# algbio/GraphChainer

Measured on AMD Instinct MI355X. Metric: reads_per_sec, higher is better.
Workload: dtype u64

## Files before the change

### graphchainer_amd/csrc/hip/gc_device.hpp

```cpp
#pragma once
#include <hip/hip_runtime.h>
#include <stdint.h>

#ifndef GC_LOOP_TICK
#define GC_LOOP_TICK(i) ((void)0)
#endif

namespace gcdev {

struct NodeRec {
	uint32_t comp;
	uint32_t outOff;
	uint32_t inOff;
	uint32_t meta;
	uint64_t w0, w1;
};
enum : uint32_t { NODEREC_SLOW = 128u };

struct DGraph {
	uint32_t nNodes;
	uint32_t firstAmbiguous;
	const uint8_t*  nodeLength;
	const uint32_t* nodeOffset;
	const int32_t*  nodeIDs;
	const uint64_t* nodeSeq;
	const uint64_t* ambSeq;
	const uint32_t* inOff;  const uint32_t* inAdj;
	const uint32_t* outOff; const uint32_t* outAdj;
	const uint32_t* componentNumber;
	const uint32_t* origSize;
	const uint32_t* lookupOff;
	const uint32_t* lookup;
	const uint32_t* componentMap;
	const uint32_t* topoId;
	const uint32_t* pathsOff; const uint32_t* paths; const uint32_t* pathsPos;
	const uint32_t* backOff;  const uint32_t* backNode; const uint32_t* backPath; const uint32_t* backPos;
	const uint32_t* mpcWidth;
	const uint32_t* chainNumber;
	const uint64_t* chainApproxPos;
	const NodeRec* nodeRec;
};

struct WS {
	uint64_t VP, VN;
	int32_t score;
};

__device__ __forceinline__ int popc64(uint64_t x) { return __popcll(x); }
__device__ __forceinline__ int32_t wsBefore(const WS& w) { return w.score - popc64(w.VP) + popc64(w.VN); }
__device__ __forceinline__ int32_t wsValue(const WS& w, int row)
{
	uint64_t above = row < 63 ? (~0ull << (row + 1)) : 0ull;
	return w.score + popc64(w.VN & above) - popc64(w.VP & above);
}

__device__ inline WS wsMerge(const WS& a, const WS& b)
{
	int32_t d = wsBefore(a) - wsBefore(b);
	uint64_t takeB = 0, fixP = 0, fixN = 0, fixMask = 0;
	uint64_t diff = (a.VP ^ b.VP) | (a.VN ^ b.VN);
	int pos = 0;
	while (diff) {
		GC_LOOP_TICK(0);
		int r = __ffsll((long long)diff) - 1;
		diff &= diff - 1;
		uint64_t bit = 1ull << r;
		if (d > 0 && r > pos) takeB |= (bit - 1) & ~((1ull << pos) - 1);
		int da = (int)((a.VP >> r) & 1) - (int)((a.VN >> r) & 1);
		int db = (int)((b.VP >> r) & 1) - (int)((b.VN >> r) & 1);
		int nd = d + da - db;
		bool before = d > 0, after = nd > 0;
		if (before != after) {
			int delta = after ? (db - d) : (da + d);
			fixMask |= bit;
			if (delta > 0) fixP |= bit;
// ... 175 lines not shown
	uint32_t startBit;
	__device__ __forceinline__ void rows(int len, int j, Eq4& eq) const;
};
__device__ inline void eqVectorBits(const EqSource& src, int len, int j, Eq4& eq)
{
	int n = len - j;
	if (n > 64) n = 64;
	uint32_t bit = src.startBit + (uint32_t)j;
	uint32_t w = bit >> 6, sh = bit & 63;
	uint64_t keep = n >= 64 ? ~0ull : ((1ull << n) - 1);
	uint64_t out[4];
	for (int b = 0; b < 4; b++) {
		const uint64_t* v = src.masks + (size_t)b * src.words;
		uint64_t lo = v[w] >> sh;
		uint64_t hi = (sh != 0 && w + 1 < src.words) ? (v[w + 1] << (64 - sh)) : 0ull;
		out[b] = (lo | hi) & keep;
	}
	eq.a = out[0]; eq.c = out[1]; eq.g = out[2]; eq.t = out[3];
}
__device__ __forceinline__ void EqSource::rows(int len, int j, Eq4& eq) const { eqVectorBits(*this, len, j, eq); }

struct NodeSeq { uint64_t w0, w1, w2, w3; bool ambiguous; };
__device__ __forceinline__ NodeSeq loadNodeSeq(const DGraph& g, uint32_t node)
{
	NodeSeq s;
	if (node < g.firstAmbiguous) {
		s.w0 = g.nodeSeq[2 * (size_t)node];
		s.w1 = g.nodeSeq[2 * (size_t)node + 1];
		s.w2 = s.w3 = 0;
		s.ambiguous = false;
	} else {
		const uint64_t* p = g.ambSeq + 4 * (size_t)(node - g.firstAmbiguous);
		s.w0 = p[0]; s.w1 = p[1]; s.w2 = p[2]; s.w3 = p[3];
		s.ambiguous = true;
	}
	return s;
}
__device__ __forceinline__ uint64_t eqOfColumn(const Eq4& eq, const NodeSeq& s, int pos)
{
	if (!s.ambiguous) {
		uint64_t w = pos < 32 ? s.w0 : s.w1;
		uint32_t code = (uint32_t)(w >> ((pos & 31) * 2));
		uint64_t lo = (code & 1) ? eq.c : eq.a;
		uint64_t hi = (code & 1) ? eq.t : eq.g;
		return (code & 2) ? hi : lo;
	}
	uint64_t r = 0;
	r |= ((s.w0 >> pos) & 1) ? eq.a : 0ull;
	r |= ((s.w1 >> pos) & 1) ? eq.c : 0ull;
	r |= ((s.w2 >> pos) & 1) ? eq.g : 0ull;
	r |= ((s.w3 >> pos) & 1) ? eq.t : 0ull;
	return r;
}

__device__ inline int findItem(const uint32_t* itemNodes, const SliceInfo& sl, uint32_t node)
{
	for (uint32_t i = 0; i < sl.count; i++)
		if (itemNodes[sl.first + i] == node) return (int)(sl.first + i);
	return -1;
}

__device__ __forceinline__ int32_t clipXScore(int32_t cells, int32_t scoreHere, double errorCost)
{
#pragma clang fp contract(off)
	const double product = (double)scoreHere * errorCost;
	const double difference = (double)cells - product;
// ... 586 lines not shown
```

### graphchainer_amd/csrc/hip/gc_device_wave.hpp

```cpp
#pragma once
#include "gc_device.hpp"
#include "gc_column_asm.hpp"
#include <type_traits>

namespace gcdev {


#ifndef WAVE_CAP
#define WAVE_CAP 28
#endif

#define WAVE_ENTRY_WORDS 7
#define WAVE_WORDS (3 * WAVE_CAP * WAVE_ENTRY_WORDS)
template <int LANES> struct WaveLdsT { uint32_t w[WAVE_WORDS][LANES]; };
typedef WaveLdsT<64> WaveLds;
static_assert(sizeof(WaveLds) <= 160 * 1024, "WaveLds must fit the CU's LDS");
static_assert(64 * 5 <= WAVE_WORDS, "the 64 backtrace columns (5 words each) alias the lane's table words");

#define WAVE_SPILL 228
#define WAVE_MAX_ENTRIES (WAVE_CAP + WAVE_SPILL)
#define WAVE_SPILL_WORDS (3 * WAVE_SPILL * 4)

typedef __attribute__((address_space(3))) uint32_t lds_u32;

// ... 268 lines not shown
	const int32_t beforeMin = beforeA < beforeB ? beforeA : beforeB;
	int32_t above = __builtin_amdgcn_update_dpp(0, m, 0x138, 0xf, 0xf, false);
	if (threadIdx.x == 0) above = beforeMin;
	WS res;
	res.VP = __ballot(m == above + 1);
	res.VN = __ballot(m == above - 1);
	res.score = a.score < b.score ? a.score : b.score;
	return res;
}
#endif

struct TilePreamble { uint64_t prevHP, prevHN, forceEq; int forceUntil; };
template <bool ROWS_IN_LANES>
__device__ __forceinline__ int32_t clipMaxXScoreWave(const WS& w, double errorCost)
{
#if defined(__HIP_DEVICE_COMPILE__)
	if (ROWS_IN_LANES) {
		const uint64_t upTo = ~(~1ull << threadIdx.x);
		const int32_t value = wsBefore(w) + popc64(w.VP & upTo) - popc64(w.VN & upTo);
		int32_t x = clipXScore((int32_t)threadIdx.x + 1, value, errorCost);
		auto higher = [](int32_t a, int32_t b) { return a > b ? a : b; };
		x = higher(x, __builtin_amdgcn_update_dpp(INT32_MIN, x, 0x111, 0xf, 0xf, false));
		x = higher(x, __builtin_amdgcn_update_dpp(INT32_MIN, x, 0x112, 0xf, 0xf, false));
		x = higher(x, __builtin_amdgcn_update_dpp(INT32_MIN, x, 0x114, 0xf, 0xf, false));
		x = higher(x, __builtin_amdgcn_update_dpp(INT32_MIN, x, 0x118, 0xf, 0xf, false));
		x = higher(x, __builtin_amdgcn_update_dpp(INT32_MIN, x, 0x142, 0xa, 0xf, false));
		x = higher(x, __builtin_amdgcn_update_dpp(INT32_MIN, x, 0x143, 0xc, 0xf, false));
		return (int32_t)GC_READLANE(x, 63);
	}
#endif
	return clipMaxXScore(w, errorCost, 64);
}
template <int MODE, bool CLIP = false, typename LANE_TABLES>
__device__ __forceinline__ TileResult computeTileW(const DGraph& g, uint32_t node, WS ws, bool prevExists, int32_t prevStartScore, uint64_t prevHP, uint64_t prevHN,
	const Eq4& eq, NodeItem& out, const LANE_TABLES& tables, int flatRows, uint32_t& status, TilePreamble* preambleOnly = nullptr, double errorCost = 0, int32_t* maxX = nullptr)
{
	constexpr bool COLUMNS = MODE == 1;
	int nodeLength = g.nodeLength[node];
	NodeSeq seq = loadNodeSeq(g, node);
	TileResult r;
	r.minScore = ws.score;
	r.minOffset = 0;
	if (CLIP && maxX) *maxX = clipMaxXScoreWave<LANE_TABLES::eqInLanes>(ws, errorCost);
#if defined(__HIP_DEVICE_COMPILE__)
	if (prevExists && wsBefore(ws) > prevStartScore) ws = LANE_TABLES::eqInLanes ? wsMergeWave(ws, wsSource(prevStartScore)) : wsMerge(ws, wsSource(prevStartScore));
#else
	if (prevExists && wsBefore(ws) > prevStartScore) ws = wsMerge(ws, wsSource(prevStartScore));
#endif
	int forceUntil = 0;
	if (prevExists) {
		int32_t scoreBefore = wsBefore(ws);
		int32_t scoreComparison = prevStartScore;
		if (scoreBefore > scoreComparison) status = EXT_ASSERT;
		if (scoreBefore < scoreComparison) {
			for (int fix = 1; fix < 64; fix++) {
				int32_t next = scoreComparison + (int32_t)((prevHP >> fix) & 1) - (int32_t)((prevHN >> fix) & 1);
				uint64_t mask = 1ull << fix;
				if (scoreBefore > next) status = EXT_ASSERT;
				if (scoreBefore < next) { prevHP |= mask; prevHN &= ~mask; forceUntil = fix; }
				if (scoreBefore == next) { prevHP &= ~mask; prevHN &= ~mask; }
				scoreBefore++;
				scoreComparison = next;
				if (scoreBefore >= scoreComparison) break;
			}
		}
	} else {
		forceUntil = nodeLength;
	}
	out.node = node;
	out.sVP = ws.VP; out.sVN = ws.VN; out.sScore = ws.score;
	uint64_t flatMask = flatRows > 0 ? ~(~0ull << flatRows) : 0;
	r.flatMin = INT32_MAX;
// ... 59 lines not shown
		if (ws.score < r.minScore) { r.minScore = ws.score; r.minOffset = (uint32_t)pos; }
		if (flatRows > 0) {
			int32_t f = ws.score - popc64(ws.VP & ~flatMask) + popc64(ws.VN & ~flatMask);
			if (f < r.flatMin) { r.flatMin = f; r.flatOffset = (uint32_t)pos; }
		}
		if (MODE != 0) tables.colSet((uint32_t)pos, ws);
		if (CLIP && maxX) { const int32_t x = clipMaxXScoreWave<LANE_TABLES::eqInLanes>(ws, errorCost); *maxX = x > *maxX ? x : *maxX; }
		HP |= hp << pos;
		HN |= hn << pos;
	}
	out.HP = HP; out.HN = HN;
	out.eVP = ws.VP; out.eVN = ws.VN; out.eScore = ws.score;
	return r;
}


template <bool REGCOLS, bool BAND = false, bool CLIP = false>
__device__ __forceinline__ uint32_t extendSeedWave(const DGraph& g, const CorrectnessTables& ct, const EqSource& eqSrc, int bandwidthCfg, lds_u32* lds, const WaveScratch& wsx,
	int len, uint32_t startNode, uint32_t startOffset, uint32_t which, uint32_t& nTrace, int32_t& score, ExtCounters& cnt, int rampBandwidth = 0, uint32_t maxCells = ~0u, bool forceGlobal = false,
	double errorCost = 0, int32_t xDrop = 0)
{
	static_assert(BAND || !CLIP, "CLIP is instantiated with BAND");
	const LaneLdsT<REGCOLS> L { lds, wsx.lane, wsx.lanes, wsx.spillBase(), {}, wsx.regCap < 64 ? wsx.regCap : 64u, { 0, 0, 0, 0, 0 }, 0, 0 };
	uint32_t status = EXT_OK;
	nTrace = 0;
	score = 0;
	cnt.extensions++;
	cnt.flattenTie = 0;
	int numSlices = (len + 63) / 64;
	if ((uint32_t)numSlices + 1 > wsx.maxSlices) return EXT_OVERFLOW;
	int buf = 0;
	uint32_t nPrev = 1;
	{
		int nl = g.nodeLength[startNode];
		NodeItem it;
		it.node = startNode;
		it.sVP = it.sVN = it.eVP = it.eVN = 0;
		it.sScore = (int32_t)startOffset;
		it.eScore = nl - 1 - (int32_t)startOffset;
		it.minScore = 0;
		uint64_t upToOffset = startOffset >= 63 ? ~0ull : ((1ull << (startOffset + 1)) - 1);
		uint64_t nodeMask = nl >= 64 ? ~0ull : ((1ull << nl) - 1);
		it.HN = upToOffset & ~1ull;
		it.HP = nodeMask & ~upToOffset;
		storeItem(wsx, 0, it);
		L.pSet(0, 0, startNode, it.sScore, 0, it.HP, it.HN);
		WSlice s0;
		s0.minScore = 0; s0.minNode = startNode; s0.minOffset = startOffset; s0.first = 0; s0.count = 1; s0.bandwidth = 1; s0.j = -64; s0.flags = 1;
		if (CLIP) setClipScore(s0, startNode, 0);
		storeSlice(wsx, 0, s0);
	}
	uint32_t nItems = 1, nSlices = 1;
	const bool storeCols = REGCOLS && wsx.maxCols > 0;
	uint32_t nCols = 0;
	GC_MARK_START();
	int32_t prevMinScore = 0, prevBandwidth = 1, prevJ = -64;
	double prevCorrect = ct.initCorrect, prevFalse = ct.initFalse;
	int rampUntil = 0, rampRedoIndex = -1;
	const bool rampOn = BAND && rampBandwidth > bandwidthCfg;
	const bool keepAll = BAND && forceGlobal;
	double snapCorrect = 0, snapFalse = 0;
	uint32_t snapCols = 0;
	const bool xDropOn = CLIP && xDrop > 0;
	int32_t bestXScore = 0;
	Eq4 eq;
	for (int slice = 0; slice < numSlices; slice++) {
		int j = prevJ + 64;
		eqVectorBits(eqSrc, len, j, eq);
		int32_t previousQuitScore = prevMinScore + prevBandwidth;
		int bandwidth = bandwidthCfg;
		if (BAND && rampOn && rampUntil >= slice && !xDropOn) bandwidth = rampBandwidth;
		const uint32_t sliceCols = nCols;
		uint32_t cells = 0;
		int flatRows = (!CLIP && j + 64 > len) ? (len - j) : 0;
		int32_t sliceMaxX = INT32_MIN; uint32_t sliceMaxXNode = 0xffffffffu;
		const int cb = REGCOLS ? 1 : (buf ^ 1);
		auto prevFind = [&](uint32_t node) __attribute__((always_inline)) -> int { return L.find((uint32_t)(REGCOLS ? 0 : buf), nPrev, node); };
		uint32_t nPending = 0;
		auto pushEdge = [&](uint32_t target, WS incoming, bool skipFirst) __attribute__((always_inline)) {
			int found = L.find(2u, nPending, target);
			uint32_t slot = found >= 0 ? (uint32_t)found : nPending;
			WS add = incoming;
			if (!skipFirst) {
				int pi = prevFind(target);
				bool prevExists = pi >= 0;
				int32_t prevStart = prevExists ? L.pStart(buf, (uint32_t)pi) : 0;
				uint64_t hinP, hinN;
				if (prevExists) {
					int32_t before = wsBefore(incoming);
					if (prevStart < before) { hinP = 0; hinN = 1; }
					else if (prevStart > before) { hinP = 1; hinN = 0; }
					else { hinP = 0; hinN = 0; }
				} else { hinP = 1; hinN = 0; }
				NodeSeq nseq = loadNodeSeq(g, target);
				uint64_t hp, hn;
#if defined(__HIP_DEVICE_COMPILE__)
				uint64_t eqFirst;
				if (REGCOLS && !nseq.ambiguous) {
					uint64_t lo, hi;
					const uint32_t code = (uint32_t)__builtin_amdgcn_readfirstlane((int)(uint32_t)nseq.w0);
					const uint64_t mA = gcUniform64(eq.a), mC = gcUniform64(eq.c), mG = gcUniform64(eq.g), mT = gcUniform64(eq.t);
					asm("s_bitcmp1_b32 %3, 0\n\ts_cselect_b64 %0, %5, %4\n\ts_cselect_b64 %1, %7, %6\n\ts_bitcmp1_b32 %3, 1\n\ts_cselect_b64 %2, %1, %0"
						: "=&s"(lo), "=&s"(hi), "=&s"(eqFirst) : "s"(code), "s"(mA), "s"(mC), "s"(mG), "s"(mT) : "scc");
				} else eqFirst = eqOfColumn(eq, nseq, 0);
				add = myersStep(eqFirst, incoming, hinP, hinN, hp, hn);
#else
				add = myersStep(eqOfColumn(eq, nseq, 0), incoming, hinP, hinN, hp, hn);
#endif
				if (!prevExists || wsBefore(add) < prevStart) { add.VP &= ~1ull; add.VN |= 1ull; }
			}
			if (slot == nPending) {
				if (nPending >= L.maxEntries()) { status = EXT_LDS_CAP; return; }
				L.qSet(slot, target, g.componentNumber[target], add);
				nPending++;
			} else {
#if defined(__HIP_DEVICE_COMPILE__)
				L.qSetWs(slot, REGCOLS ? wsMergeWave(L.qWs(slot), add) : wsMerge(L.qWs(slot), add));
#else
				L.qSetWs(slot, wsMerge(L.qWs(slot), add));
#endif
			}
		};
		for (uint32_t i = 0; i < nPrev; i++) {
			if (j != 0 && L.pMin(buf, i) > previousQuitScore) continue;
			pushEdge(L.pNode(buf, i), wsSource(L.pStart(buf, i)), true);
		}
		if (status != EXT_OK) return status;
		GC_MARK(0);
		WSlice cur;
		cur.first = nItems; cur.count = 0; cur.bandwidth = bandwidth; cur.j = j;
		cur.minScore = INT32_MAX - bandwidth - 1; cur.minNode = 0xffffffffu; cur.minOffset = 0xffffffffu;
		int32_t flatMin = INT32_MAX; uint32_t flatNode = 0xffffffffu, flatOffset = 0xffffffffu;
		int32_t currentMin = cur.minScore;
		while (nPending > 0) {
			const uint32_t best = L.qArgMin(nPending);
			uint32_t pnode = L.qNode(best);
			WS pws = L.qWs(best);
			if (best != nPending - 1) L.qMove(best, nPending - 1);
			nPending--;
			if (nItems >= wsx.maxItems) return EXT_OVERFLOW;
			if (cur.count >= L.maxEntries()) return EXT_LDS_CAP;
			int pi = prevFind(pnode);
			bool prevExists = pi >= 0;
			NodeItem out;
			typename LaneLdsT<REGCOLS>::Entry pe { 0, 0, 0, ~0ull, 0ull };
			if (prevExists) pe = L.get((uint32_t)buf, (uint32_t)pi);
			GC_MARK(1);
			const uint32_t tileLength = g.nodeLength[pnode];
			if (storeCols && nCols + tileLength - 1 > wsx.maxCols) return EXT_OVERFLOW;
			int32_t tileMaxX = INT32_MIN;
			TileResult tr = storeCols ? computeTileW<2, CLIP>(g, pnode, pws, prevExists, (int32_t)pe.w1, pe.a, pe.b, eq, out, L, flatRows, status, nullptr, errorCost, CLIP ? &tileMaxX : nullptr)
				: computeTileW<0, CLIP>(g, pnode, pws, prevExists, (int32_t)pe.w1, pe.a, pe.b, eq, out, L, flatRows, status, nullptr, errorCost, CLIP ? &tileMaxX : nullptr);
			GC_MARK(2);
			if (status != EXT_OK) return status;
			if (CLIP && tileMaxX > sliceMaxX) { sliceMaxX = tileMaxX; sliceMaxXNode = pnode; }
			out.minScore = tr.minScore;
			if (storeCols) {
				if (threadIdx.x >= 1 && threadIdx.x < tileLength) {
					ulonglong2 v;
					v.x = (unsigned long long)L.cr[0] | ((unsigned long long)L.cr[1] << 32);
					v.y = (unsigned long long)L.cr[2] | ((unsigned long long)L.cr[3] << 32);
					*(ulonglong2*)(wsx.base + wsx.colBase() + 2ull * (nCols + threadIdx.x - 1)) = v;
				}
				NodeItem stored = out;
				stored.minScore = (int32_t)nCols;
				storeItem(wsx, nItems, stored);
				nCols += tileLength - 1;
			} else storeItem(wsx, nItems, out);
			L.pSet(cb, cur.count, pnode, out.sScore, out.minScore, out.HP, out.HN);
			nItems++;
			cur.count++;
			cnt.dpTiles++;
			cnt.columnSteps += g.nodeLength[pnode];
			if (flatRows > 0) { cnt.recomputeTiles++; cnt.columnSteps += g.nodeLength[pnode]; }
			if (tr.minScore > previousQuitScore + bandwidth + 128) return EXT_ASSERT;
			currentMin = tr.minScore < currentMin ? tr.minScore : currentMin;
			if (tr.minScore < cur.minScore) { cur.minScore = tr.minScore; cur.minNode = pnode; cur.minOffset = tr.minOffset; }
			if (flatRows > 0) {
				if (tr.flatMin < flatMin) { flatMin = tr.flatMin; flatNode = pnode; flatOffset = tr.flatOffset; }
				else if (tr.flatMin == flatMin) flatOffset |= 0x80000000u;
			}
			WS newEnd = itemEnd(out);
#if defined(__HIP_DEVICE_COMPILE__)
			int32_t newEndMin;
			if (REGCOLS) {
				const uint64_t upTo = ~(~1ull << threadIdx.x);
				const int32_t before = wsBefore(newEnd);
				uint32_t v = (uint32_t)(before + popc64(newEnd.VP & upTo) - popc64(newEnd.VN & upTo));
				auto lower = [](uint32_t a, uint32_t b) { return (int32_t)a < (int32_t)b ? a : b; };
				v = lower(v, (uint32_t)__builtin_amdgcn_update_dpp(0x7fffffff, (int)v, 0x111, 0xf, 0xf, false));
				v = lower(v, (uint32_t)__builtin_amdgcn_update_dpp(0x7fffffff, (int)v, 0x112, 0xf, 0xf, false));
				v = lower(v, (uint32_t)__builtin_amdgcn_update_dpp(0x7fffffff, (int)v, 0x114, 0xf, 0xf, false));
				v = lower(v, (uint32_t)__builtin_amdgcn_update_dpp(0x7fffffff, (int)v, 0x118, 0xf, 0xf, false));
				v = lower(v, (uint32_t)__builtin_amdgcn_update_dpp(0x7fffffff, (int)v, 0x142, 0xa, 0xf, false));
				v = lower(v, (uint32_t)__builtin_amdgcn_update_dpp(0x7fffffff, (int)v, 0x143, 0xc, 0xf, false));
				const int32_t rowsMin = (int32_t)GC_READLANE(v, 63);
				newEndMin = rowsMin < before ? rowsMin : before;
			} else newEndMin = wsColumnMin(newEnd);
#else
			int32_t newEndMin = wsColumnMin(newEnd);
#endif
			if (newEndMin < prevMinScore) return EXT_ASSERT;
			if (newEndMin <= currentMin + bandwidth) {
				GC_MARK(3);
				for (uint32_t e = g.outOff[pnode]; e < g.outOff[pnode + 1]; e++) {
					pushEdge(g.outAdj[e], newEnd, false);
					if (status != EXT_OK) return status;
				}
				GC_MARK(4);
			} else GC_MARK(3);
			if (BAND) {
				cells += tileLength;
				if (cells > maxCells) break;
			}
		}
		GC_MARK(1);
		if (cur.count == 0) return EXT_ASSERT;
		const uint32_t flatTie = flatRows > 0 ? (flatOffset >> 31) << 3 : 0u;
		if (flatRows > 0) { cur.minScore = flatMin; cur.minNode = flatNode; cur.minOffset = flatOffset & 0x7fffffffu; }
		if (cur.minScore < prevMinScore) return EXT_ASSERT;
		if (CLIP) setClipScore(cur, sliceMaxXNode, sliceMaxX + j);
		double curCorrect, curFalse;
		{
			int mm = cur.minScore - prevMinScore;
			int idx = mm < 64 ? mm : 63;
			bool cfc = prevCorrect + ct.c2c >= prevFalse + ct.f2c;
			bool ffc = prevCorrect + ct.c2f >= prevFalse + ct.f2f;
			double a = prevCorrect + ct.c2c, b = prevFalse + ct.f2c;
			double c = prevCorrect + ct.c2f, d = prevFalse + ct.f2f;
			curCorrect = (a > b ? a : b) + ct.correctOdds[idx];
			curFalse = (c > d ? c : d) + ct.wrongOdds[idx];
			cur.flags = (curCorrect > curFalse ? 1u : 0u) | (cfc ? 2u : 0u) | (ffc ? 4u : 0u) | flatTie;
		}
		if (BAND) {
			if (!keepAll && !xDropOn && (rampUntil == slice - 1 || (rampUntil < slice && (cur.flags & 1u) && (cur.flags & 4u)))) {
				if (nPrev > wsx.maxTrace) return EXT_OVERFLOW;
				rampRedoIndex = slice - 1;
				snapCorrect = prevCorrect; snapFalse = prevFalse; snapCols = sliceCols;
				for (uint32_t i = 0; i < nPrev; i++) { const int32_t mn = L.pMin(buf, i); if (wsx.storer()) wsx.word(wsx.traceBase(i, which)) = (unsigned long long)(uint32_t)mn; }
// ... 70 lines not shown
		if (REGCOLS) {
			const bool mine = threadIdx.x == (nTrace & 63u);
			tbLo = mine ? (uint32_t)cell : tbLo;
			tbHi = mine ? (uint32_t)(cell >> 32) : tbHi;
			nTrace++;
			if ((nTrace & 63u) == 0) flushTrace(64);
		} else {
			wsx.word(wsx.traceBase(nTrace, which)) = cell;
			nTrace++;
		}
		return true;
	};
	Cell here { last.minNode, last.minOffset, (last.j + 63 < len - 1) ? last.j + 63 : len - 1 };
	if (CLIP) {
		uint32_t bestIndex = 1;
		WSlice bs = loadSlice(wsx, 1);
		for (uint32_t k = 2; k < nSlices; k++) { const WSlice t = loadSlice(wsx, k); if (clipScore(t) > clipScore(bs)) { bs = t; bestIndex = k; } }
		const uint32_t bestNode = clipNode(bs);
		const int bestItem = findItemW(wsx, bs, bestNode);
		if (bestItem < 0) return EXT_ASSERT;
		const NodeItem it = loadItem(wsx, (uint32_t)bestItem);
		const int prevIdx = findItemW(wsx, loadSlice(wsx, bestIndex - 1), bestNode);
		const bool prevExists = prevIdx >= 0;
		NodeItem pit {};
		if (prevExists) pit = loadItem(wsx, (uint32_t)prevIdx);
		eqVectorBits(eqSrc, len, bs.j, eq);
		ClipFind find { clipScore(bs) - bs.j, len - bs.j < 64 ? len - bs.j : 64, false, 0u, 0, 0 };
		NodeItem scratch;
		computeTile<true>(g, bestNode, itemStart(it), prevExists, prevExists ? pit.sScore : 0, prevExists ? pit.HP : ~0ull, prevExists ? pit.HN : 0ull,
			eq, scratch, nullptr, 0, status, 63, 1, 63, errorCost, nullptr, &find);
		if (scratch.eVP != it.eVP || scratch.eVN != it.eVN || scratch.eScore != it.eScore) status = EXT_ASSERT;
		if (status != EXT_OK) return status;
		cnt.recomputeTiles++;
		cnt.columnSteps += g.nodeLength[bestNode];
		if (!find.found) return EXT_ASSERT;
		here = Cell { bestNode, find.column, bs.j + find.row };
		score = find.value;
	}
	if (!pushTraceW(here, false)) return status;
	uint32_t curSliceIdx = 0xffffffffu, curNode = 0xffffffffu;
	WSlice cs = last, ps = last;
	const uint32_t ID_CACHE = 64, idsCurBase = 64 * 5, idsPrevBase = 64 * 5 + ID_CACHE;
	static_assert(64 * 5 + 2 * 64 <= WAVE_WORDS, "id caches must fit behind the backtrace columns");
	auto fillIds = [&](const WSlice& sl, uint32_t base) __attribute__((always_inline)) {
		if (REGCOLS) {
			uint32_t id = 0xffffffffu;
			if (threadIdx.x < sl.count) id = (uint32_t)wsx.base[(wsx.itemBase(sl.first + threadIdx.x) + 7) * wsx.lanes + wsx.lane];
			if (base == idsCurBase) L.idCur = id; else L.idPrev = id;
			return;
		}
		uint32_t n = sl.count < ID_CACHE ? sl.count : ID_CACHE;
		for (uint32_t i = 0; i < n; i++) L.stL(base + i, itemNode(wsx, sl.first + i));
	};
	auto findIn = [&](const WSlice& sl, uint32_t base, uint32_t node) __attribute__((always_inline)) -> int {
		if (REGCOLS) {
			unsigned long long m = base == idsCurBase ? __ballot(L.idCur == node) : __ballot(L.idPrev == node);
			if (sl.count < 64) m &= (1ull << sl.count) - 1;
			return m ? (int)(sl.first + (uint32_t)__ffsll((long long)m) - 1) : -1;
		}
		if (sl.count > ID_CACHE) return findItemW(wsx, sl, node);
		for (uint32_t i = 0; i < sl.count; i++) if (L.ldL(base + i) == node) return (int)(sl.first + i);
		return -1;
	};
	auto findCur = [&](uint32_t node) __attribute__((always_inline)) -> int { return findIn(cs, idsCurBase, node); };
	auto findPrev = [&](uint32_t node) __attribute__((always_inline)) -> int { return findIn(ps, idsPrevBase, node); };
	NodeItem curIt {};
	NodeItem prevIt {};
	bool prevItExists = false;
	auto corner = [&](Cell& out, bool& nodeSwitch) __attribute__((always_inline)) -> bool {
		GC_MARK(10);
		struct MarkOnExit { ExtCounters& cnt; __device__ ~MarkOnExit() { GC_MARK(9); } } markOnExit { cnt };
		int32_t j = cs.j;
		int32_t quitScore = cs.minScore + cs.bandwidth;
		int32_t previousQuitScore = ps.minScore + ps.bandwidth;
		int32_t scoreHere = wsValue(itemStart(curIt), 0);
		uint32_t inBegin = g.inOff[curNode], inEnd = g.inOff[curNode + 1];
		if (scoreHere > quitScore) {
			int32_t smallest = scoreHere + 1;
			out = Cell { 0, 0, 0 };
			nodeSwitch = false;
			if (prevItExists) { smallest = prevIt.sScore; out = Cell { curNode, 0, j - 1 }; }
			for (uint32_t e = inBegin; e < inEnd; e++) {
				uint32_t nb = g.inAdj[e];
				int p = findPrev(nb);
				if (p >= 0) { NodeItem pn = loadItem(wsx, (uint32_t)p); if (pn.eScore <= smallest) { smallest = pn.eScore; out = Cell { nb, (uint32_t)g.nodeLength[nb] - 1, j - 1 }; nodeSwitch = true; } }
				int c = findCur(nb);
				if (c >= 0 && nb != curNode) {
					int32_t v = wsValue(itemEnd(loadItem(wsx, (uint32_t)c)), 0);
					if (v < smallest) { smallest = v; out = Cell { nb, (uint32_t)g.nodeLength[nb] - 1, j }; nodeSwitch = true; }
				}
			}
			return true;
		}
		NodeSeq nseq = loadNodeSeq(g, curNode);
		int eqBit = (int)(eqOfColumn(eq, nseq, 0) & 1);
		if (prevItExists && prevIt.sScore == scoreHere - 1) { out = Cell { curNode, 0, j - 1 }; nodeSwitch = false; return true; }
		Cell bestInvalid { 0xffffffffu, 0xffffffffu, -1 };
		int32_t bestInvalidScore = scoreHere + 1;
		for (uint32_t e = inBegin; e < inEnd; e++) {
			uint32_t nb = g.inAdj[e];
			int c = findCur(nb);
			if (c >= 0 && wsValue(itemEnd(loadItem(wsx, (uint32_t)c)), 0) == scoreHere - 1) { out = Cell { nb, (uint32_t)g.nodeLength[nb] - 1, j }; nodeSwitch = true; return true; }
			int p = findPrev(nb);
			if (p >= 0) {
				int32_t cornerScore = loadItem(wsx, (uint32_t)p).eScore;
				if (cornerScore > previousQuitScore) {
					if (cornerScore < bestInvalidScore) { bestInvalidScore = cornerScore; bestInvalid = Cell { nb, (uint32_t)g.nodeLength[nb] - 1, j - 1 }; }
				} else if (cornerScore == scoreHere - (eqBit ? 0 : 1)) {
					out = Cell { nb, (uint32_t)g.nodeLength[nb] - 1, j - 1 }; nodeSwitch = true; return true;
				}
			}
		}
		if (bestInvalidScore < scoreHere + 1) { out = bestInvalid; nodeSwitch = true; return true; }
		return false;
	};
	while (here.seqPos != -1) {
		uint32_t s = (uint32_t)(here.seqPos / 64) + 1;
		if (s >= nSlices) return EXT_ASSERT;
		if (s != curSliceIdx || here.node != curNode) {
			GC_MARK(10);
			if (s != curSliceIdx) { cs = loadSlice(wsx, s); ps = loadSlice(wsx, s - 1); eqVectorBits(eqSrc, len, cs.j, eq); fillIds(cs, idsCurBase); fillIds(ps, idsPrevBase); }
			GC_MARK(6);
			curSliceIdx = s;
			curNode = here.node;
			int ci = findCur(curNode);
			if (ci < 0) return EXT_ASSERT;
			curIt = loadItem(wsx, (uint32_t)ci);
			int pi = findPrev(curNode);
			prevItExists = pi >= 0;
			if (prevItExists) prevIt = loadItem(wsx, (uint32_t)pi);
			GC_MARK(7);
			NodeItem scratchItem;
#if defined(__HIP_DEVICE_COMPILE__)
			if (storeCols) {
				TilePreamble pre;
				computeTileW<1>(g, curNode, itemStart(curIt), prevItExists, prevItExists ? prevIt.sScore : 0, prevItExists ? prevIt.HP : ~0ull, prevItExists ? prevIt.HN : 0ull,
					eq, scratchItem, L, 0, status, &pre);
				const uint32_t tileLength = g.nodeLength[curNode];
				const uint32_t c = threadIdx.x;
				unsigned long long vp = curIt.sVP, vn = curIt.sVN;
				if (c >= 1 && c < tileLength) {
					const ulonglong2 v = *(const ulonglong2*)(wsx.base + wsx.colBase() + 2ull * ((uint32_t)curIt.minScore + c - 1));
					vp = v.x; vn = v.y;
				}
				L.cr[0] = (uint32_t)vp; L.cr[1] = (uint32_t)(vp >> 32); L.cr[2] = (uint32_t)vn; L.cr[3] = (uint32_t)(vn >> 32);
				const uint64_t upToC = (c >= 63 ? ~0ull : ((2ull << c) - 1)) & ~1ull;
				L.cr[4] = (uint32_t)(curIt.sScore + popc64(curIt.HP & upToC) - popc64(curIt.HN & upToC));
				const NodeSeq seq = loadNodeSeq(g, curNode);
				L.walkMasks = false;
				if (!seq.ambiguous) L.setWalkMasks(seq.w0, seq.w1, eq, pre.forceEq, pre.prevHN);
			} else
#endif
			{
				computeTileW<1>(g, curNode, itemStart(curIt), prevItExists, prevItExists ? prevIt.sScore : 0, prevItExists ? prevIt.HP : ~0ull, prevItExists ? prevIt.HN : 0ull,
					eq, scratchItem, L, 0, status);
				if (scratchItem.eVP != curIt.eVP || scratchItem.eVN != curIt.eVN || scratchItem.eScore != curIt.eScore) status = EXT_ASSERT;
			}
			cnt.recomputeTiles++; cnt.backtraceTiles++; cnt.columnSteps += g.nodeLength[curNode];
			if (status != EXT_OK) return status;
			GC_MARK(8);
		}
		int row = here.seqPos & 63;
		if (row == 0 && here.offset == 0) {
			Cell nxt; bool sw;
			if (!corner(nxt, sw)) return EXT_ASSERT;
			if (!pushTraceW(nxt, sw)) return status;
			here = nxt;
			continue;
		}
		if (row == 0) {
			if (!prevItExists) {
				here = Cell { curNode, 0, here.seqPos };
				if (!pushTraceW(here, false)) return status;
				continue;
			}
			uint32_t off = here.offset;
			while (off > 0 && wsValue(L.col(off - 1), 0) == wsValue(L.col(off), 0) - 1) {
				off--;
				if (!pushTraceW(Cell { curNode, off, here.seqPos }, false)) return status;
			}
			here.offset = off;
			if (off == 0) {
				Cell nxt; bool sw;
				if (!corner(nxt, sw)) return EXT_ASSERT;
				if (!pushTraceW(nxt, sw)) return status;
				here = nxt;
				continue;
			}
			int32_t scoreHere = wsValue(L.col(off), 0);
			int32_t scoreDiagonal = prevIt.sScore;
			uint64_t lowMask = ((1ull << off) - 1) & ~1ull;
			scoreDiagonal += popc64(prevIt.HP & lowMask) - popc64(prevIt.HN & lowMask);
			int32_t scoreUp = scoreDiagonal + (int32_t)((prevIt.HP >> off) & 1) - (int32_t)((prevIt.HN >> off) & 1);
			int32_t quitScore = cs.minScore + cs.bandwidth, previousQuitScore = ps.minScore + ps.bandwidth;
			Cell nxt;
			if (scoreHere > quitScore || scoreDiagonal > previousQuitScore || scoreUp > previousQuitScore) {
				nxt = scoreDiagonal < scoreUp ? Cell { curNode, off - 1, here.seqPos - 1 } : Cell { curNode, off, here.seqPos - 1 };
			} else {
				NodeSeq nseq = loadNodeSeq(g, curNode);
				int eqBit = (int)(eqOfColumn(eq, nseq, (int)off) & 1);
				if (scoreUp == scoreHere - 1) nxt = Cell { curNode, off, here.seqPos - 1 };
				else if (scoreDiagonal == scoreHere - (eqBit ? 0 : 1)) nxt = Cell { curNode, off - 1, here.seqPos - 1 };
				else return EXT_ASSERT;
			}
			if (!pushTraceW(nxt, false)) return status;
			here = nxt;
			continue;
		}
		if (here.offset == 0) {
			WS start = itemStart(curIt);
			int32_t sp = here.seqPos;
			while ((sp & 63) != 0 && (start.VP & (1ull << (sp & 63)))) {
				sp--;
				if (!pushTraceW(Cell { curNode, 0, sp }, false)) return status;
			}
			here.seqPos = sp;
			int offset = sp & 63;
			if (offset == 0) {
				Cell nxt; bool sw;
				if (!corner(nxt, sw)) return EXT_ASSERT;
				if (!pushTraceW(nxt, sw)) return status;
				here = nxt;
				continue;
			}
			NodeSeq nseq = loadNodeSeq(g, curNode);
			int eqBit = (int)((eqOfColumn(eq, nseq, 0) >> offset) & 1);
			int32_t scoreHere = wsValue(start, offset);
			int32_t quitScore = cs.minScore + cs.bandwidth;
			Cell nxt { 0, 0, 0 };
			bool sw = false, found = false;
			if (scoreHere > quitScore) {
				int32_t smallest = wsValue(start, offset - 1);
				nxt = Cell { curNode, 0, sp - 1 };
				for (uint32_t e = g.inOff[curNode]; e < g.inOff[curNode + 1]; e++) {
					uint32_t nb = g.inAdj[e];
					int c = findCur(nb);
					if (c < 0) continue;
					WS ne = itemEnd(loadItem(wsx, (uint32_t)c));
					if (wsValue(ne, offset - 1) <= smallest) { smallest = wsValue(ne, offset - 1); nxt = Cell { nb, (uint32_t)g.nodeLength[nb] - 1, sp - 1 }; sw = true; }
					if (wsValue(ne, offset) < smallest && nb != curNode) { smallest = wsValue(ne, offset); nxt = Cell { nb, (uint32_t)g.nodeLength[nb] - 1, sp }; sw = true; }
				}
				found = true;
			} else {
				for (uint32_t e = g.inOff[curNode]; e < g.inOff[curNode + 1] && !found; e++) {
					uint32_t nb = g.inAdj[e];
					int c = findCur(nb);
					if (c < 0) continue;
					WS ne = itemEnd(loadItem(wsx, (uint32_t)c));
					if (wsValue(ne, offset) == scoreHere - 1) { nxt = Cell { nb, (uint32_t)g.nodeLength[nb] - 1, sp }; sw = true; found = true; }
					else if (wsValue(ne, offset - 1) == scoreHere - (eqBit ? 0 : 1)) { nxt = Cell { nb, (uint32_t)g.nodeLength[nb] - 1, sp - 1 }; sw = true; found = true; }
				}
			}
			if (!found) return EXT_ASSERT;
			if (!pushTraceW(nxt, sw)) return status;
			here = nxt;
			continue;
		}
#if defined(__HIP_DEVICE_COMPILE__)
		if (REGCOLS && L.walkMasks) {
			uint32_t hori = here.offset;
			int vert = row;
			uint64_t up, diag, left;
			L.loadWalkMasks(hori, up, diag, left);
			uint32_t unfit = 0;
			while (hori > 0 && vert > 0) {
				{
					const int dgn = (int)hori - vert;
					const int myRow = (int)threadIdx.x - dgn;
					const uint64_t myUp = (uint64_t)L.cr[0] | ((uint64_t)L.cr[1] << 32), myDiag = (uint64_t)L.wm[0] | ((uint64_t)L.wm[1] << 32);
					const bool diagonalStep = threadIdx.x >= 1 && myRow >= 1 && myRow < 64 && ((myDiag >> (myRow & 63)) & 1ull) && !((myUp >> (myRow & 63)) & 1ull);
					const uint64_t runMask = __ballot(diagonalStep);
					const uint64_t stops = ~runMask & (hori >= 63 ? ~0ull : ((2ull << hori) - 1));
					const uint32_t firstStop = 63u - (uint32_t)__builtin_clzll(stops);
					const uint32_t run = hori - firstStop;
					if (run > 0) {
						uint32_t remaining = run, k0 = 0;
						while (remaining) {
							const uint32_t slot0 = nTrace & 63u;
							const uint32_t take = remaining < 64u - slot0 ? remaining : 64u - slot0;
							if (threadIdx.x >= slot0 && threadIdx.x < slot0 + take) {
								const uint32_t k = k0 + (threadIdx.x - slot0);
								const unsigned long long cell = packCell(Cell { curNode, hori - 1 - k, cs.j + vert - 1 - (int)k }, false);
								tbLo = (uint32_t)cell; tbHi = (uint32_t)(cell >> 32);
							}
							nTrace += take; remaining -= take; k0 += take;
							if ((nTrace & 63u) == 0) {
								if (nTrace > wsx.maxTrace) return EXT_OVERFLOW;
								wsx.base[(wsx.traceBase(nTrace - 64, which)) * wsx.lanes + wsx.lane + threadIdx.x] = (unsigned long long)tbLo | ((unsigned long long)tbHi << 32);
							}
						}
						hori -= run; vert -= (int)run;
						if (hori > 0 && vert > 0) L.loadWalkMasks(hori, up, diag, left);
						continue;
					}
				}
				const uint32_t u = (uint32_t)(up >> vert) & 1u, d = (uint32_t)(diag >> vert) & 1u, l = (uint32_t)(left >> vert) & 1u;
				unfit |= (u | d | l) ^ 1u;
				vert -= (int)(u | d);
				if (!u) { hori--; L.loadWalkMasks(hori, up, diag, left); }
				if (!pushTraceW(Cell { curNode, hori, cs.j + vert }, false)) return status;
			}
			if (unfit) return EXT_ASSERT;
			here = Cell { curNode, hori, cs.j + vert };
		} else if (REGCOLS) {
			uint32_t hori = here.offset;
			int vert = row;
			const NodeSeq nseq = loadNodeSeq(g, curNode);
			const uint32_t laneRow = threadIdx.x;
			const uint64_t above = ~1ull << laneRow;
			auto rowValues = [&](const WS& c) __attribute__((always_inline)) -> int32_t { return c.score - popc64(c.VP & above) + popc64(c.VN & above); };
			WS ch = L.col(hori);
			int32_t av = rowValues(ch);
			while (hori > 0 && vert > 0) {
				const WS cl = L.col(hori - 1);
				const int32_t bv = rowValues(cl);
				const int32_t bUp = __builtin_amdgcn_update_dpp(0, bv, 0x138, 0xf, 0xf, false);
				const uint64_t diagSame = __ballot(bUp == av), diagLess = __ballot(bUp == av - 1), leftFits = __ballot(bv == av - 1);
				uint64_t eqColumn = eqOfColumn(eq, nseq, (int)hori);
				eqColumn = (uint64_t)(uint32_t)__builtin_amdgcn_readfirstlane((int)(uint32_t)eqColumn) | ((uint64_t)(uint32_t)__builtin_amdgcn_readfirstlane((int)(uint32_t)(eqColumn >> 32)) << 32);
				const uint64_t diagFits = (diagSame & eqColumn) | (diagLess & ~eqColumn);
				bool moved = false;
				do {
					const uint64_t bit = 1ull << vert;
					if (ch.VP & bit) vert--;
					else if (diagFits & bit) { hori--; vert--; moved = true; }
					else {
						if (!(leftFits & bit)) return EXT_ASSERT;
						hori--;
						moved = true;
					}
					if (!pushTraceW(Cell { curNode, hori, cs.j + vert }, false)) return status;
				} while (!moved && vert > 0);
				if (moved) { ch = cl; av = bv; }
			}
			here = Cell { curNode, hori, cs.j + vert };
		} else
#endif
		{
			uint32_t hori = here.offset;
			int vert = row;
			NodeSeq nseq = loadNodeSeq(g, curNode);
			WS ch = L.col(hori), cl = L.col(hori - 1);
			int32_t scoreHere = wsValue(ch, vert), leftHere = wsValue(cl, vert);
			while (hori > 0 && vert > 0) {
				int32_t vertical = scoreHere - (int32_t)((ch.VP >> vert) & 1) + (int32_t)((ch.VN >> vert) & 1);
				int32_t diagonal = leftHere - (int32_t)((cl.VP >> vert) & 1) + (int32_t)((cl.VN >> vert) & 1);
				int eqBit = (int)((eqOfColumn(eq, nseq, (int)hori) >> vert) & 1);
				bool left = false;
				if (vertical == scoreHere - 1) { vert--; scoreHere = vertical; leftHere = diagonal; }
				else if (diagonal == scoreHere - (eqBit ? 0 : 1)) { hori--; vert--; scoreHere = diagonal; left = true; }
				else {
					if (leftHere != scoreHere - 1) return EXT_ASSERT;
					hori--;
					scoreHere = leftHere;
					left = true;
				}
				if (left) {
					ch = cl;
					if (hori > 0) { cl = L.col(hori - 1); leftHere = wsValue(cl, vert); }
				}
				if (!pushTraceW(Cell { curNode, hori, cs.j + vert }, false)) return status;
			}
			here = Cell { curNode, hori, cs.j + vert };
		}
	}
	{
		if (here.node != startNode) return EXT_ASSERT;
		uint32_t off = here.offset;
		while (true) {
			int32_t b = (int32_t)off - (int32_t)startOffset; if (b < 0) b = -b;
			int32_t bl = (int32_t)off - 1 - (int32_t)startOffset; if (bl < 0) bl = -bl;
			if (!(b != 0 && off > 0 && bl == b - 1)) break;
			off--;
			if (!pushTraceW(Cell { here.node, off, -1 }, false)) return status;
// ... 12 lines not shown
```

Measured before the change: 76060.

## Read packed per-node records via constant address space in wave extension

Replaces the separate per-node lookups of length, sequence words, component number and edge offsets with a single 32-byte NodeRec load. The load goes through the constant address space, so the compiler can emit scalar loads for the wave-uniform node. Edge ranges come from degree fields packed into the record, with a fallback to the offset array for high-degree nodes. The aim is fewer scattered global memory transactions per tile and edge push. The cost is the extra meta decode and the assumption that the record array is built consistently on the host.

```diff
diff --git a/graphchainer_amd/csrc/hip/gc_device.hpp b/graphchainer_amd/csrc/hip/gc_device.hpp
--- a/graphchainer_amd/csrc/hip/gc_device.hpp
+++ b/graphchainer_amd/csrc/hip/gc_device.hpp
@@ -41,6 +41,45 @@
 	const NodeRec* nodeRec;
 };
 
+template <typename T> __device__ __forceinline__ T gcK(const T* p)
+{
+#if defined(__HIP_DEVICE_COMPILE__)
+	return *(const __attribute__((address_space(4))) T*)(unsigned long long)p;
+#else
+	return *p;
+#endif
+}
+__device__ __forceinline__ NodeRec gcNodeRec(const DGraph& g, uint32_t node)
+{
+#if defined(__HIP_DEVICE_COMPILE__)
+	typedef uint32_t Words8 __attribute__((ext_vector_type(8)));
+	static_assert(sizeof(NodeRec) == sizeof(Words8), "NodeRec is eight words");
+	const Words8 w = gcK((const Words8*)(g.nodeRec + node));
+	NodeRec r;
+	r.comp = w[0]; r.outOff = w[1]; r.inOff = w[2]; r.meta = w[3];
+	r.w0 = (uint64_t)w[4] | ((uint64_t)w[5] << 32); r.w1 = (uint64_t)w[6] | ((uint64_t)w[7] << 32);
+	return r;
+#else
+	return g.nodeRec[node];
+#endif
+}
+__device__ __forceinline__ uint32_t recLength(const NodeRec& r) { return r.meta & 127u; }
+__device__ __forceinline__ uint32_t recRank(const NodeRec& r) { return r.comp; }
+__device__ __forceinline__ uint32_t gcNodeLength(const DGraph& g, uint32_t node) { return gcK(&g.nodeRec[node].meta) & 127u; }
+struct EdgeRange { uint32_t begin, end; };
+__device__ __forceinline__ EdgeRange recOutRange(const DGraph& g, uint32_t node, const NodeRec& r)
+{
+	const uint32_t deg = (r.meta >> 8) & 255u;
+	return EdgeRange { r.outOff, deg < 255u ? r.outOff + deg : gcK(g.outOff + node + 1) };
+}
+__device__ __forceinline__ EdgeRange recInRange(const DGraph& g, uint32_t node, const NodeRec& r)
+{
+	const uint32_t deg = (r.meta >> 16) & 255u;
+	return EdgeRange { r.inOff, deg < 255u ? r.inOff + deg : gcK(g.inOff + node + 1) };
+}
+__device__ __forceinline__ uint32_t gcOutAdj(const DGraph& g, uint32_t e) { return gcK(g.outAdj + e); }
+__device__ __forceinline__ uint32_t gcInAdj(const DGraph& g, uint32_t e) { return gcK(g.inAdj + e); }
+
 struct WS {
 	uint64_t VP, VN;
 	int32_t score;
@@ -282,6 +321,20 @@
 	} else {
 		const uint64_t* p = g.ambSeq + 4 * (size_t)(node - g.firstAmbiguous);
 		s.w0 = p[0]; s.w1 = p[1]; s.w2 = p[2]; s.w3 = p[3];
+		s.ambiguous = true;
+	}
+	return s;
+}
+__device__ __forceinline__ NodeSeq recNodeSeq(const DGraph& g, uint32_t node, const NodeRec& r)
+{
+	NodeSeq s;
+	if (!(r.meta & NODEREC_SLOW)) {
+		s.w0 = r.w0; s.w1 = r.w1;
+		s.w2 = s.w3 = 0;
+		s.ambiguous = false;
+	} else {
+		const uint64_t* p = g.ambSeq + 4 * (size_t)(node - g.firstAmbiguous);
+		s.w0 = gcK(p); s.w1 = gcK(p + 1); s.w2 = gcK(p + 2); s.w3 = gcK(p + 3);
 		s.ambiguous = true;
 	}
 	return s;
diff --git a/graphchainer_amd/csrc/hip/gc_device_wave.hpp b/graphchainer_amd/csrc/hip/gc_device_wave.hpp
--- a/graphchainer_amd/csrc/hip/gc_device_wave.hpp
+++ b/graphchainer_amd/csrc/hip/gc_device_wave.hpp
@@ -324,12 +324,12 @@
 	return clipMaxXScore(w, errorCost, 64);
 }
 template <int MODE, bool CLIP = false, typename LANE_TABLES>
-__device__ __forceinline__ TileResult computeTileW(const DGraph& g, uint32_t node, WS ws, bool prevExists, int32_t prevStartScore, uint64_t prevHP, uint64_t prevHN,
+__device__ __forceinline__ TileResult computeTileW(const DGraph& g, uint32_t node, const NodeRec& rec, WS ws, bool prevExists, int32_t prevStartScore, uint64_t prevHP, uint64_t prevHN,
 	const Eq4& eq, NodeItem& out, const LANE_TABLES& tables, int flatRows, uint32_t& status, TilePreamble* preambleOnly = nullptr, double errorCost = 0, int32_t* maxX = nullptr)
 {
 	constexpr bool COLUMNS = MODE == 1;
-	int nodeLength = g.nodeLength[node];
-	NodeSeq seq = loadNodeSeq(g, node);
+	int nodeLength = (int)recLength(rec);
+	NodeSeq seq = recNodeSeq(g, node, rec);
 	TileResult r;
 	r.minScore = ws.score;
 	r.minOffset = 0;
@@ -455,7 +455,7 @@
 	int buf = 0;
 	uint32_t nPrev = 1;
 	{
-		int nl = g.nodeLength[startNode];
+		int nl = (int)gcNodeLength(g, startNode);
 		NodeItem it;
 		it.node = startNode;
 		it.sVP = it.sVN = it.eVP = it.eVN = 0;
@@ -501,6 +501,7 @@
 		auto prevFind = [&](uint32_t node) __attribute__((always_inline)) -> int { return L.find((uint32_t)(REGCOLS ? 0 : buf), nPrev, node); };
 		uint32_t nPending = 0;
 		auto pushEdge = [&](uint32_t target, WS incoming, bool skipFirst) __attribute__((always_inline)) {
+			const NodeRec trec = gcNodeRec(g, target);
 			int found = L.find(2u, nPending, target);
 			uint32_t slot = found >= 0 ? (uint32_t)found : nPending;
 			WS add = incoming;
@@ -515,7 +516,7 @@
 					else if (prevStart > before) { hinP = 1; hinN = 0; }
 					else { hinP = 0; hinN = 0; }
 				} else { hinP = 1; hinN = 0; }
-				NodeSeq nseq = loadNodeSeq(g, target);
+				NodeSeq nseq = recNodeSeq(g, target, trec);
 				uint64_t hp, hn;
 #if defined(__HIP_DEVICE_COMPILE__)
 				uint64_t eqFirst;
@@ -534,7 +535,7 @@
 			}
 			if (slot == nPending) {
 				if (nPending >= L.maxEntries()) { status = EXT_LDS_CAP; return; }
-				L.qSet(slot, target, g.componentNumber[target], add);
+				L.qSet(slot, target, recRank(trec), add);
 				nPending++;
 			} else {
 #if defined(__HIP_DEVICE_COMPILE__)
@@ -569,11 +570,12 @@
 			typename LaneLdsT<REGCOLS>::Entry pe { 0, 0, 0, ~0ull, 0ull };
 			if (prevExists) pe = L.get((uint32_t)buf, (uint32_t)pi);
 			GC_MARK(1);
-			const uint32_t tileLength = g.nodeLength[pnode];
+			const NodeRec prec = gcNodeRec(g, pnode);
+			const uint32_t tileLength = recLength(prec);
 			if (storeCols && nCols + tileLength - 1 > wsx.maxCols) return EXT_OVERFLOW;
 			int32_t tileMaxX = INT32_MIN;
-			TileResult tr = storeCols ? computeTileW<2, CLIP>(g, pnode, pws, prevExists, (int32_t)pe.w1, pe.a, pe.b, eq, out, L, flatRows, status, nullptr, errorCost, CLIP ? &tileMaxX : nullptr)
-				: computeTileW<0, CLIP>(g, pnode, pws, prevExists, (int32_t)pe.w1, pe.a, pe.b, eq, out, L, flatRows, status, nullptr, errorCost, CLIP ? &tileMaxX : nullptr);
+			TileResult tr = storeCols ? computeTileW<2, CLIP>(g, pnode, prec, pws, prevExists, (int32_t)pe.w1, pe.a, pe.b, eq, out, L, flatRows, status, nullptr, errorCost, CLIP ? &tileMaxX : nullptr)
+				: computeTileW<0, CLIP>(g, pnode, prec, pws, prevExists, (int32_t)pe.w1, pe.a, pe.b, eq, out, L, flatRows, status, nullptr, errorCost, CLIP ? &tileMaxX : nullptr);
 			GC_MARK(2);
 			if (status != EXT_OK) return status;
 			if (CLIP && tileMaxX > sliceMaxX) { sliceMaxX = tileMaxX; sliceMaxXNode = pnode; }
@@ -594,8 +596,8 @@
 			nItems++;
 			cur.count++;
 			cnt.dpTiles++;
-			cnt.columnSteps += g.nodeLength[pnode];
-			if (flatRows > 0) { cnt.recomputeTiles++; cnt.columnSteps += g.nodeLength[pnode]; }
+			cnt.columnSteps += tileLength;
+			if (flatRows > 0) { cnt.recomputeTiles++; cnt.columnSteps += tileLength; }
 			if (tr.minScore > previousQuitScore + bandwidth + 128) return EXT_ASSERT;
 			currentMin = tr.minScore < currentMin ? tr.minScore : currentMin;
 			if (tr.minScore < cur.minScore) { cur.minScore = tr.minScore; cur.minNode = pnode; cur.minOffset = tr.minOffset; }
@@ -626,8 +628,9 @@
 			if (newEndMin < prevMinScore) return EXT_ASSERT;
 			if (newEndMin <= currentMin + bandwidth) {
 				GC_MARK(3);
-				for (uint32_t e = g.outOff[pnode]; e < g.outOff[pnode + 1]; e++) {
-					pushEdge(g.outAdj[e], newEnd, false);
+				const EdgeRange outs = recOutRange(g, pnode, prec);
+				for (uint32_t e = outs.begin; e < outs.end; e++) {
+					pushEdge(gcOutAdj(g, e), newEnd, false);
 					if (status != EXT_OK) return status;
 				}
 				GC_MARK(4);
@@ -764,7 +767,7 @@
 		if (scratch.eVP != it.eVP || scratch.eVN != it.eVN || scratch.eScore != it.eScore) status = EXT_ASSERT;
 		if (status != EXT_OK) return status;
 		cnt.recomputeTiles++;
-		cnt.columnSteps += g.nodeLength[bestNode];
+		cnt.columnSteps += gcNodeLength(g, bestNode);
 		if (!find.found) return EXT_ASSERT;
 		here = Cell { bestNode, find.column, bs.j + find.row };
 		score = find.value;
@@ -806,40 +809,42 @@
 		int32_t quitScore = cs.minScore + cs.bandwidth;
 		int32_t previousQuitScore = ps.minScore + ps.bandwidth;
 		int32_t scoreHere = wsValue(itemStart(curIt), 0);
-		uint32_t inBegin = g.inOff[curNode], inEnd = g.inOff[curNode + 1];
+		const NodeRec crec = gcNodeRec(g, curNode);
+		const EdgeRange ins = recInRange(g, curNode, crec);
+		const uint32_t inBegin = ins.begin, inEnd = ins.end;
 		if (scoreHere > quitScore) {
 			int32_t smallest = scoreHere + 1;
 			out = Cell { 0, 0, 0 };
 			nodeSwitch = false;
 			if (prevItExists) { smallest = prevIt.sScore; out = Cell { curNode, 0, j - 1 }; }
 			for (uint32_t e = inBegin; e < inEnd; e++) {
-				uint32_t nb = g.inAdj[e];
+				uint32_t nb = gcInAdj(g, e);
 				int p = findPrev(nb);
-				if (p >= 0) { NodeItem pn = loadItem(wsx, (uint32_t)p); if (pn.eScore <= smallest) { smallest = pn.eScore; out = Cell { nb, (uint32_t)g.nodeLength[nb] - 1, j - 1 }; nodeSwitch = true; } }
+				if (p >= 0) { NodeItem pn = loadItem(wsx, (uint32_t)p); if (pn.eScore <= smallest) { smallest = pn.eScore; out = Cell { nb, gcNodeLength(g, nb) - 1, j - 1 }; nodeSwitch = true; } }
 				int c = findCur(nb);
 				if (c >= 0 && nb != curNode) {
 					int32_t v = wsValue(itemEnd(loadItem(wsx, (uint32_t)c)), 0);
-					if (v < smallest) { smallest = v; out = Cell { nb, (uint32_t)g.nodeLength[nb] - 1, j }; nodeSwitch = true; }
+					if (v < smallest) { smallest = v; out = Cell { nb, gcNodeLength(g, nb) - 1, j }; nodeSwitch = true; }
 				}
 			}
 			return true;
 		}
-		NodeSeq nseq = loadNodeSeq(g, curNode);
+		NodeSeq nseq = recNodeSeq(g, curNode, crec);
 		int eqBit = (int)(eqOfColumn(eq, nseq, 0) & 1);
 		if (prevItExists && prevIt.sScore == scoreHere - 1) { out = Cell { curNode, 0, j - 1 }; nodeSwitch = false; return true; }
 		Cell bestInvalid { 0xffffffffu, 0xffffffffu, -1 };
 		int32_t bestInvalidScore = scoreHere + 1;
 		for (uint32_t e = inBegin; e < inEnd; e++) {
-			uint32_t nb = g.inAdj[e];
+			uint32_t nb = gcInAdj(g, e);
 			int c = findCur(nb);
-			if (c >= 0 && wsValue(itemEnd(loadItem(wsx, (uint32_t)c)), 0) == scoreHere - 1) { out = Cell { nb, (uint32_t)g.nodeLength[nb] - 1, j }; nodeSwitch = true; return true; }
+			if (c >= 0 && wsValue(itemEnd(loadItem(wsx, (uint32_t)c)), 0) == scoreHere - 1) { out = Cell { nb, gcNodeLength(g, nb) - 1, j }; nodeSwitch = true; return true; }
 			int p = findPrev(nb);
 			if (p >= 0) {
 				int32_t cornerScore = loadItem(wsx, (uint32_t)p).eScore;
 				if (cornerScore > previousQuitScore) {
-					if (cornerScore < bestInvalidScore) { bestInvalidScore = cornerScore; bestInvalid = Cell { nb, (uint32_t)g.nodeLength[nb] - 1, j - 1 }; }
+					if (cornerScore < bestInvalidScore) { bestInvalidScore = cornerScore; bestInvalid = Cell { nb, gcNodeLength(g, nb) - 1, j - 1 }; }
 				} else if (cornerScore == scoreHere - (eqBit ? 0 : 1)) {
-					out = Cell { nb, (uint32_t)g.nodeLength[nb] - 1, j - 1 }; nodeSwitch = true; return true;
+					out = Cell { nb, gcNodeLength(g, nb) - 1, j - 1 }; nodeSwitch = true; return true;
 				}
 			}
 		}
@@ -863,12 +868,13 @@
 			if (prevItExists) prevIt = loadItem(wsx, (uint32_t)pi);
 			GC_MARK(7);
 			NodeItem scratchItem;
+			const NodeRec curRec = gcNodeRec(g, curNode);
 #if defined(__HIP_DEVICE_COMPILE__)
 			if (storeCols) {
 				TilePreamble pre;
-				computeTileW<1>(g, curNode, itemStart(curIt), prevItExists, prevItExists ? prevIt.sScore : 0, prevItExists ? prevIt.HP : ~0ull, prevItExists ? prevIt.HN : 0ull,
+				computeTileW<1>(g, curNode, curRec, itemStart(curIt), prevItExists, prevItExists ? prevIt.sScore : 0, prevItExists ? prevIt.HP : ~0ull, prevItExists ? prevIt.HN : 0ull,
 					eq, scratchItem, L, 0, status, &pre);
-				const uint32_t tileLength = g.nodeLength[curNode];
+				const uint32_t tileLength = recLength(curRec);
 				const uint32_t c = threadIdx.x;
 				unsigned long long vp = curIt.sVP, vn = curIt.sVN;
 				if (c >= 1 && c < tileLength) {
@@ -878,17 +884,17 @@
 				L.cr[0] = (uint32_t)vp; L.cr[1] = (uint32_t)(vp >> 32); L.cr[2] = (uint32_t)vn; L.cr[3] = (uint32_t)(vn >> 32);
 				const uint64_t upToC = (c >= 63 ? ~0ull : ((2ull << c) - 1)) & ~1ull;
 				L.cr[4] = (uint32_t)(curIt.sScore + popc64(curIt.HP & upToC) - popc64(curIt.HN & upToC));
-				const NodeSeq seq = loadNodeSeq(g, curNode);
+				const NodeSeq seq = recNodeSeq(g, curNode, curRec);
 				L.walkMasks = false;
 				if (!seq.ambiguous) L.setWalkMasks(seq.w0, seq.w1, eq, pre.forceEq, pre.prevHN);
 			} else
 #endif
 			{
-				computeTileW<1>(g, curNode, itemStart(curIt), prevItExists, prevItExists ? prevIt.sScore : 0, prevItExists ? prevIt.HP : ~0ull, prevItExists ? prevIt.HN : 0ull,
+				computeTileW<1>(g, curNode, curRec, itemStart(curIt), prevItExists, prevItExists ? prevIt.sScore : 0, prevItExists ? prevIt.HP : ~0ull, prevItExists ? prevIt.HN : 0ull,
 					eq, scratchItem, L, 0, status);
 				if (scratchItem.eVP != curIt.eVP || scratchItem.eVN != curIt.eVN || scratchItem.eScore != curIt.eScore) status = EXT_ASSERT;
 			}
-			cnt.recomputeTiles++; cnt.backtraceTiles++; cnt.columnSteps += g.nodeLength[curNode];
+			cnt.recomputeTiles++; cnt.backtraceTiles++; cnt.columnSteps += recLength(curRec);
 			if (status != EXT_OK) return status;
 			GC_MARK(8);
 		}
@@ -929,7 +935,7 @@
 			if (scoreHere > quitScore || scoreDiagonal > previousQuitScore || scoreUp > previousQuitScore) {
 				nxt = scoreDiagonal < scoreUp ? Cell { curNode, off - 1, here.seqPos - 1 } : Cell { curNode, off, here.seqPos - 1 };
 			} else {
-				NodeSeq nseq = loadNodeSeq(g, curNode);
+				NodeSeq nseq = recNodeSeq(g, curNode, gcNodeRec(g, curNode));
 				int eqBit = (int)(eqOfColumn(eq, nseq, (int)off) & 1);
 				if (scoreUp == scoreHere - 1) nxt = Cell { curNode, off, here.seqPos - 1 };
 				else if (scoreDiagonal == scoreHere - (eqBit ? 0 : 1)) nxt = Cell { curNode, off - 1, here.seqPos - 1 };
@@ -955,7 +961,9 @@
 				here = nxt;
 				continue;
 			}
-			NodeSeq nseq = loadNodeSeq(g, curNode);
+			const NodeRec crec = gcNodeRec(g, curNode);
+			const EdgeRange ins = recInRange(g, curNode, crec);
+			NodeSeq nseq = recNodeSeq(g, curNode, crec);
 			int eqBit = (int)((eqOfColumn(eq, nseq, 0) >> offset) & 1);
 			int32_t scoreHere = wsValue(start, offset);
 			int32_t quitScore = cs.minScore + cs.bandwidth;
@@ -964,23 +972,23 @@
 			if (scoreHere > quitScore) {
 				int32_t smallest = wsValue(start, offset - 1);
 				nxt = Cell { curNode, 0, sp - 1 };
-				for (uint32_t e = g.inOff[curNode]; e < g.inOff[curNode + 1]; e++) {
-					uint32_t nb = g.inAdj[e];
+				for (uint32_t e = ins.begin; e < ins.end; e++) {
+					uint32_t nb = gcInAdj(g, e);
 					int c = findCur(nb);
 					if (c < 0) continue;
 					WS ne = itemEnd(loadItem(wsx, (uint32_t)c));
-					if (wsValue(ne, offset - 1) <= smallest) { smallest = wsValue(ne, offset - 1); nxt = Cell { nb, (uint32_t)g.nodeLength[nb] - 1, sp - 1 }; sw = true; }
-					if (wsValue(ne, offset) < smallest && nb != curNode) { smallest = wsValue(ne, offset); nxt = Cell { nb, (uint32_t)g.nodeLength[nb] - 1, sp }; sw = true; }
+					if (wsValue(ne, offset - 1) <= smallest) { smallest = wsValue(ne, offset - 1); nxt = Cell { nb, gcNodeLength(g, nb) - 1, sp - 1 }; sw = true; }
+					if (wsValue(ne, offset) < smallest && nb != curNode) { smallest = wsValue(ne, offset); nxt = Cell { nb, gcNodeLength(g, nb) - 1, sp }; sw = true; }
 				}
 				found = true;
 			} else {
-				for (uint32_t e = g.inOff[curNode]; e < g.inOff[curNode + 1] && !found; e++) {
-					uint32_t nb = g.inAdj[e];
+				for (uint32_t e = ins.begin; e < ins.end && !found; e++) {
+					uint32_t nb = gcInAdj(g, e);
 					int c = findCur(nb);
 					if (c < 0) continue;
 					WS ne = itemEnd(loadItem(wsx, (uint32_t)c));
-					if (wsValue(ne, offset) == scoreHere - 1) { nxt = Cell { nb, (uint32_t)g.nodeLength[nb] - 1, sp }; sw = true; found = true; }
-					else if (wsValue(ne, offset - 1) == scoreHere - (eqBit ? 0 : 1)) { nxt = Cell { nb, (uint32_t)g.nodeLength[nb] - 1, sp - 1 }; sw = true; found = true; }
+					if (wsValue(ne, offset) == scoreHere - 1) { nxt = Cell { nb, gcNodeLength(g, nb) - 1, sp }; sw = true; found = true; }
+					else if (wsValue(ne, offset - 1) == scoreHere - (eqBit ? 0 : 1)) { nxt = Cell { nb, gcNodeLength(g, nb) - 1, sp - 1 }; sw = true; found = true; }
 				}
 			}
 			if (!found) return EXT_ASSERT;
@@ -1037,7 +1045,7 @@
 		} else if (REGCOLS) {
 			uint32_t hori = here.offset;
 			int vert = row;
-			const NodeSeq nseq = loadNodeSeq(g, curNode);
+			const NodeSeq nseq = recNodeSeq(g, curNode, gcNodeRec(g, curNode));
 			const uint32_t laneRow = threadIdx.x;
 			const uint64_t above = ~1ull << laneRow;
 			auto rowValues = [&](const WS& c) __attribute__((always_inline)) -> int32_t { return c.score - popc64(c.VP & above) + popc64(c.VN & above); };
@@ -1071,7 +1079,7 @@
 		{
 			uint32_t hori = here.offset;
 			int vert = row;
-			NodeSeq nseq = loadNodeSeq(g, curNode);
+			NodeSeq nseq = recNodeSeq(g, curNode, gcNodeRec(g, curNode));
 			WS ch = L.col(hori), cl = L.col(hori - 1);
 			int32_t scoreHere = wsValue(ch, vert), leftHere = wsValue(cl, vert);
 			while (hori > 0 && vert > 0) {
```

After: 79110, median of 6. 1.04x the previous value.
